# hkchengrex/Cutie

Measured on AMD Instinct MI355X. Metric: frames/sec (480p, 3 objects), higher is better.
Workload: dtype bf16

## Files before the change

cutie_amd/_lib.py:

```python
import ctypes
import os

_HERE = os.path.dirname(os.path.abspath(__file__))
LIB_PATH = os.environ.get('CUTIE_AMD_LIB') or os.path.join(_HERE, 'libcutie_hip.so')
ABI_VERSION = 9
OP_STRUCT_SIZE = 256

_lib = None


class HipLibraryError(RuntimeError):
    pass


def load():
    global _lib
    if _lib is not None:
        return _lib
    if not os.path.exists(LIB_PATH):
        raise HipLibraryError(
            f'{LIB_PATH} not found: build it with `python -c "import __graft_entry__ as g; g.build()"` '
            f'(or `make -C cutie_amd/csrc`).  cutie_amd has no CPU fallback.')
    lib = ctypes.CDLL(LIB_PATH)
    lib.cutie_exec.argtypes = [ctypes.c_void_p, ctypes.c_int, ctypes.c_void_p]
    lib.cutie_exec.restype = ctypes.c_int
    lib.cutie_exec_one.argtypes = [ctypes.c_void_p, ctypes.c_void_p]
    lib.cutie_exec_one.restype = ctypes.c_int
    lib.cutie_graph_capture.argtypes = [ctypes.c_void_p, ctypes.c_int, ctypes.c_void_p]
# ... 109 lines not shown
```

cutie_amd/csrc/api.hip:

```cpp
#include "common.h"
#include <stdarg.h>
#include <stdio.h>
#include <string.h>

static thread_local char g_err[512] = "";

void cutie_set_error(const char* fmt, ...) {
    va_list ap;
    va_start(ap, fmt);
    vsnprintf(g_err, sizeof(g_err), fmt, ap);
    va_end(ap);
}

static int dispatch(const cutie_op* op, hipStream_t s) {
    switch (op->kind) {
        case CUTIE_OP_CONV: return launch_conv(op, s);
        case CUTIE_OP_QUERY_INIT: return (op->flags & 1) ? launch_attention(op, s) : launch_elementwise(op, s);
        case CUTIE_OP_QFFN: return launch_qchain(op, s);
        case CUTIE_OP_STEM: return launch_stem(op, s);
        case CUTIE_OP_ATTN_Q2P: case CUTIE_OP_ATTN_SELF: case CUTIE_OP_ATTN_P2Q:
            return (op->flags & 12) ? launch_qchain(op, s) : launch_attention(op, s);
        case CUTIE_OP_AUX_MASK:
            return launch_attention(op, s);
        case CUTIE_OP_KEY_PREP: case CUTIE_OP_AFF_SCORE: case CUTIE_OP_AFF_SELECT: case CUTIE_OP_AFF_READOUT:
// ... 78 lines not shown
    hipGraphExecDestroy(h->exec);
    hipGraphDestroy(h->graph);
    delete h;
}

float cutie_time_ops(const cutie_op* ops, int n, int iters, void* stream) {
    hipStream_t s = (hipStream_t)stream;
    hipEvent_t a, b;
    if (hipEventCreate(&a) != hipSuccess || hipEventCreate(&b) != hipSuccess) { cutie_set_error("time: event create failed"); return -1.f; }
    if (cutie_exec(ops, n, stream) != 0) return -1.f;
    hipEventRecord(a, s);
    for (int it = 0; it < iters; ++it)
        if (cutie_exec(ops, n, stream) != 0) return -1.f;
    hipEventRecord(b, s);
    hipEventSynchronize(b);
    float ms = 0.f;
    hipEventElapsedTime(&ms, a, b);
    hipEventDestroy(a);
    hipEventDestroy(b);
    return ms / (float)iters;
}

const char* cutie_hip_last_error(void) { return g_err; }
int cutie_hip_abi_version(void) { return 9; }
int cutie_op_struct_size(void) { return (int)sizeof(cutie_op); }
int cutie_hip_build_flags(void) {
#ifdef CUTIE_DIAG
    return 1;
#else
    return 0;
#endif
}

}
```

cutie_amd/csrc/elementwise.hip:

```cpp
#include "common.h"
#include <math.h>

#define GRID1D(n, bs) dim3((unsigned)(((long)(n) + (bs) - 1) / (bs)))
__global__ void memset32_kernel(uint32_t* d, long n, uint32_t v);

__global__ void maxpool_kernel(const uint4* __restrict__ x, uint4* __restrict__ y, int B, int H, int W, int C8,
                               int OH, int OW, int relu) {
    long idx = (long)blockIdx.x * blockDim.x + threadIdx.x;
    long total = (long)B * OH * OW * C8;
    if (idx >= total) return;
    int c = idx % C8; long t = idx / C8;
    int ow = t % OW; t /= OW; int oh = t % OH; int b = t / OH;
    float m[8];
#pragma unroll
    for (int i = 0; i < 8; ++i) m[i] = relu ? 0.f : -INFINITY;
    for (int dy = 0; dy < 3; ++dy) {
        int ih = oh * 2 - 1 + dy;
        if ((unsigned)ih >= (unsigned)H) continue;
        for (int dx = 0; dx < 3; ++dx) {
            int iw = ow * 2 - 1 + dx;
            if ((unsigned)iw >= (unsigned)W) continue;
            uint4 v = x[(((long)b * H + ih) * W + iw) * C8 + c];
            uint32_t u[4] = {v.x, v.y, v.z, v.w};
#pragma unroll
// ... 344 lines not shown
                const uint32_t* xu = &xv[it].x; const uint32_t* ru = &rv[it].x;
#pragma unroll
                for (int i = 0; i < 4; ++i) {
                    const float lo = __uint_as_float(xu[i] << 16) * sc[(2 * i) * 32 + c8] + __uint_as_float(ru[i] << 16);
                    const float hi = __uint_as_float(xu[i] & 0xffff0000u) * sc[(2 * i + 1) * 32 + c8] + __uint_as_float(ru[i] & 0xffff0000u);
                    const uint32_t st = pack_bf2(lo, hi);
                    part += fmaxf(__uint_as_float(st << 16), 0.f) * __uint_as_float(wu[i] << 16);
                    part += fmaxf(__uint_as_float(st & 0xffff0000u), 0.f) * __uint_as_float(wu[i] & 0xffff0000u);
                }
            }
            part += __uint_as_float(__builtin_amdgcn_update_dpp(0, (int)__float_as_uint(part), 0xB1, 0xf, 0xf, false));
            part += __uint_as_float(__builtin_amdgcn_update_dpp(0, (int)__float_as_uint(part), 0x4E, 0xf, 0xf, false));
            part += __uint_as_float(__builtin_amdgcn_update_dpp(0, (int)__float_as_uint(part), 0x141, 0xf, 0xf, false));
            part += __uint_as_float(__builtin_amdgcn_update_dpp(0, (int)__float_as_uint(part), 0x140, 0xf, 0xf, false));
            const unsigned pu = __float_as_uint(part);
            const auto rr = __builtin_amdgcn_permlane16_swap(pu, pu, false, false);
            const float tot = __uint_as_float(rr[0]) + __uint_as_float(rr[1]);
            const int q = tid + it * 256, p = p0 + q / C8;
            if (c8 == 0 && offs[it] >= 0) plog[(long)b * HW + p] = tot + bias;
        }
    }
}

__global__ void gru4_kernel(const float* __restrict__ v, float* __restrict__ h, bf16_t* __restrict__ hb, long n, int C, int prio) {
    if (prio) __builtin_amdgcn_s_setprio(1);
    const long idx = (long)blockIdx.x * blockDim.x + threadIdx.x;
    const int C4 = C >> 2;
    if (idx >= n * C4) return;
    const long row = idx / C4; const int c = (int)(idx - row * C4) * 4;
    const float* vr = v + row * 3 * C + c;
    const float4 f4 = *reinterpret_cast<const float4*>(vr), u4 = *reinterpret_cast<const float4*>(vr + C), n4 = *reinterpret_cast<const float4*>(vr + 2 * C);
    const float4 h4 = *reinterpret_cast<const float4*>(h + row * C + c);
    const float fa[4] = {f4.x, f4.y, f4.z, f4.w}, ua[4] = {u4.x, u4.y, u4.z, u4.w}, na[4] = {n4.x, n4.y, n4.z, n4.w}, ha[4] = {h4.x, h4.y, h4.z, h4.w};
    float o[4];
#pragma unroll
    for (int i = 0; i < 4; ++i) {
        const float f = sigmoidf_(fa[i]), u = sigmoidf_(ua[i]), nv = tanhf(na[i]);
        o[i] = f * ha[i] * (1.f - u) + u * nv;
    }
    *reinterpret_cast<float4*>(h + row * C + c) = make_float4(o[0], o[1], o[2], o[3]);
    *reinterpret_cast<uint2*>(hb + row * C + c) = make_uint2(pack_bf2(o[0], o[1]), pack_bf2(o[2], o[3]));
}

__global__ void gru_kernel(const float* __restrict__ v, float* __restrict__ h, bf16_t* __restrict__ hb, long n, int C) {
    long idx = (long)blockIdx.x * blockDim.x + threadIdx.x;
    if (idx >= n * C) return;
// ... 850 lines not shown
            break;
        }
        case CUTIE_OP_MASK_DOWN: {
            int K = i[0], r = i[3], h = i[1] / r, w = i[2] / r;
            long n = (long)K * h * w;
            float* m16 = (float*)p[2];
            if (!m16) { cutie_set_error("mask_down: m16 buffer required"); return -2; }
            hipLaunchKernelGGL(mask_down_pair_kernel, GRID1D((long)h * w * 64, BS), dim3(BS), 0, s, (const float*)p[0], m16, (uint4*)p[1], K, i[1], i[2], r,
                               i[4] > 8 ? i[4] / 8 : 1);
            break;
        }
        case CUTIE_OP_GAP: {
            if (i[2] > 256 || (i[2] & 7) || 256 % (i[2] / 8)) { cutie_set_error("gap: C must divide 256 octet-wise (C=%d)", i[2]); return -2; }
            if (!p[2]) { cutie_set_error("gap: scratch buffer required"); return -2; }
            int nchunk = (i[1] + 63) / 64;
            hipLaunchKernelGGL(gap_partial_kernel, dim3(nchunk, i[0]), dim3(256), 0, s, (const bf16_t*)p[0], (float*)p[2], i[1], i[2]);
            if (!(op->flags & 1))
                hipLaunchKernelGGL(gap_final_kernel, dim3(i[0]), dim3(256), 0, s, (const float*)p[2], (float*)p[1], nchunk, i[2], 1.f / (float)i[1]);
            break;
        }
        case CUTIE_OP_ECA_APPLY: {
            if (i[2] > 256 || (i[2] & 7)) { cutie_set_error("eca: C <= 256, C %% 8"); return -2; }
            if (p[6] && (i[2] != 256 || !p[8])) { cutie_set_error("eca: the fused 1x1 head needs C = 256 and an output"); return -2; }
            int nchunk = (i[1] + 63) / 64;
            hipLaunchKernelGGL(eca_apply_kernel, dim3((i[1] + 31) / 32, i[0]), dim3(256), 0, s, (const bf16_t*)p[0], (const float*)p[5], (const float*)p[2],
                               (const bf16_t*)p[3], (bf16_t*)p[4], (float*)p[1], i[1], i[2], nchunk, (op->flags & 1) ? (const long long*)p[5] : nullptr,
                               (const bf16_t*)p[6], (const float*)p[7], (float*)p[8], PRIO);
            break;
        }
        case CUTIE_OP_GRU: {
            long n = (long)i[0] * i[1];
            if (!(op->flags & 1) && (i[1] & 3) == 0 && (((uintptr_t)p[0] | (uintptr_t)p[1]) & 15) == 0 && ((uintptr_t)p[2] & 7) == 0)
                hipLaunchKernelGGL(gru4_kernel, GRID1D(n / 4, BS), dim3(BS), 0, s, (const float*)p[0], (float*)p[1], (bf16_t*)p[2], (long)i[0], i[1], PRIO);
            else
                hipLaunchKernelGGL(gru_kernel, GRID1D(n, BS), dim3(BS), 0, s, (const float*)p[0], (float*)p[1], (bf16_t*)p[2], (long)i[0], i[1]);
            break;
        }
        case CUTIE_OP_SEG_AGG:
            hipLaunchKernelGGL(seg_agg_kernel, GRID1D(i[1], BS), dim3(BS), 0, s, (const float*)p[0], (float*)p[1], i[0], i[1]);
            break;
        case CUTIE_OP_UP4_SOFTMAX: {
            long n = (long)16 * i[1] * i[2];
            if (op->flags & 1) {
                if (i[0] > 16) { cutie_set_error("up4_softmax: the fused form holds P <= 16 planes in registers (P=%d)", i[0]); return -2; }
                const bool vec = !(op->flags & 2) && i[0] <= 8 && (((uintptr_t)p[1] | (uintptr_t)p[2]) & 15) == 0;
                const int nclip = i[4] > 1 ? i[4] : 1;
// ... 206 lines not shown
```

cutie_amd/inference/inference_core.py:

```python
import contextlib
import logging
import os
from typing import List, Optional

import numpy as np
import torch

from .. import _lib, frame_context, ops as O
from ..model import plans
from .image_feature_store import ImageFeatureStore
from .memory_manager import MemoryManager
from .object_manager import ObjectManager

log = logging.getLogger()
F32 = torch.float32
DEFER_MEM = os.environ.get('CUTIE_AMD_DEFER_MEM', '0') not in ('', '0')
WAIT_TRACE = None
AFF_BATCH = int(os.environ.get('CUTIE_AMD_AFF_BATCH', '8'))
AFF_FIRST_ALONE = os.environ.get('CUTIE_AMD_AFF_FIRST_ALONE', '1') not in ('', '0')
WINDOW = int(os.environ.get('CUTIE_AMD_WINDOW', '12'))
WINDOW_LEAD = int(os.environ.get('CUTIE_AMD_WINDOW_LEAD', '3'))


def pad_geometry(h, w, d=16):
# ... 356 lines not shown
            msk_value, finish = self.network.encode_mask(
                image, pix_feat, self.memory.get_sensory(ids), prob, deep_update=is_deep_update, chunk_size=self.chunk_size,
                need_weights=self.save_aux, _raw=raw, _split=True)
            self.memory.add_memory(key, shrinkage, msk_value, None, ids, selection=selection, as_permanent=as_permanent)
            feats = pre[2]
            ev = self._ahead_affinity(feats[2], feats[4], pre[3], self._prefetched_rec, next_mem_ti=self.curr_ti + self.mem_every, first_alone=AFF_FIRST_ALONE)
            self._prefetched = pre[:3] + (ev,) + pre[4:]
            sensory, obj_value = finish()
            self.memory.add_object_values(obj_value, ids)
        else:
            msk_value, sensory, obj_value, _ = self.network.encode_mask(
                image, pix_feat, self.memory.get_sensory(ids), prob, deep_update=is_deep_update, chunk_size=self.chunk_size,
                need_weights=self.save_aux, _raw=raw)
            self.memory.add_memory(key, shrinkage, msk_value, obj_value, ids, selection=selection, as_permanent=as_permanent)
        self.last_mem_ti = self.curr_ti
        if is_deep_update:
            self.memory.update_sensory(sensory, ids)

    def _segment(self, key, selection, pix_feat, ms_features, update_sensory=True) -> torch.Tensor:
        if not self.memory.engaged:
            log.warning('Trying to segment without any memory!')
            return torch.zeros((1, key.shape[-2] * 16, key.shape[-1] * 16), device=key.device, dtype=key.dtype)
        ids = self.object_manager.all_obj_ids
        memory_readout = self.memory.read(pix_feat, key, selection, self.last_mask, self.network)
        stacked = self.memory.readout_stacked(ids)
        memory_readout = stacked if stacked is not None else self.object_manager.realize_dict(memory_readout)
        sensory, _, pred_prob_with_bg = self.network.segment(ms_features, memory_readout, self.memory.get_sensory(ids),
                                                             chunk_size=self.chunk_size, update_sensory=update_sensory,
                                                             _need_logits=False, _fork=self._hinted)
        pred_prob_with_bg = pred_prob_with_bg[0]
        if update_sensory:
            self.memory.update_sensory(sensory, ids)
        return pred_prob_with_bg

    def step(self, image: torch.Tensor, mask: Optional[torch.Tensor] = None, objects: Optional[List[int]] = None, *,
             idx_mask: bool = True, end: bool = False, delete_buffer: bool = True, force_permanent: bool = False,
             next_image: Optional[torch.Tensor] = None, next_images=None) -> torch.Tensor:
        if objects is None and mask is not None:
            assert not idx_mask
            objects = list(range(1, mask.shape[0] + 1))

        resize_needed = False
        if self.max_internal_size > 0:
            h, w = image.shape[-2:]
            min_side = min(h, w)
            if min_side > self.max_internal_size:
                resize_needed = True
# ... 187 lines not shown
```

cutie_amd/inference/memory_manager.py:

```python
import itertools
import logging
import os
from typing import Dict, List

import torch

from .. import frame_context, ops as O
from .kv_memory_store import Bucket, StoreView, LIFE_EPS_BITS
from .object_manager import ObjectManager

log = logging.getLogger()
BF16, F32 = torch.bfloat16, torch.float32
CAND_CAP = 1024
_VALIDATE = os.environ.get('CUTIE_AMD_VALIDATE', '0') not in ('', '0')
PATCH_PLANS = os.environ.get('CUTIE_AMD_PATCH_PLANS', '1') not in ('', '0')
_VERSIONS = itertools.count(1)


class MemoryManager:
    def __init__(self, cfg, object_manager: ObjectManager):
        self.object_manager = object_manager
        self.sensory_dim = cfg.model.sensory_dim
        self.top_k = cfg.top_k
        self.chunk_size = cfg.chunk_size
# ... 407 lines not shown
                q['_readouts_joint'] = readout[e:e + C].view(C * K, h, w, m0.CV)
        return True

    def read_visual(self, q: dict, h: int, w: int, dev, network) -> Dict[int, torch.Tensor]:
        self._pool = network.engine().pool
        ahead = q.pop('_readouts', None) or {}
        ahead_ev = q.pop('_readouts_ev', None)
        if ahead_ev is not None and ahead:
            torch.cuda.current_stream(dev).wait_event(ahead_ev)
        out = {}
        for bucket in self.buckets.values():
            K = len(bucket.objects)
            pre = ahead.get(bucket.id)
            if pre is not None and pre[1] == self._version and pre[0].shape[0] == K:
                out[bucket.id] = pre[0]
                if pre[2] is not None:
                    self._commit_ahead(bucket, pre[2], network)
            else:
                self._join_side()
                out[bucket.id] = self._affinity(bucket, q, h, w, dev)
        return out

    def read(self, pix_feat: torch.Tensor, query_key: torch.Tensor, selection: torch.Tensor, last_mask: torch.Tensor,
             network) -> Dict[int, torch.Tensor]:
        q = network.query_operands(query_key, selection)
        h, w = pix_feat.shape[-2:]
        dev = pix_feat.device
        visual = self.read_visual(q, h, w, dev, network)
        all_readout = {}
        for bucket in self.buckets.values():
            K = len(bucket.objects)
            readout = visual[bucket.id]
            cs = self.chunk_size if (self.chunk_size is not None and self.chunk_size >= 1) else K
            chunks = []
            for c0 in range(0, K, cs):
                objects = bucket.objects[c0:c0 + cs]
                this_sensory = self.get_sensory(objects)
                this_last_mask = self._get_mask_by_ids(last_mask, objects)
                visual_readout = readout[c0:c0 + cs].permute(0, 3, 1, 2).unsqueeze(0)
                pixel_readout = network.pixel_fusion(pix_feat, visual_readout, this_sensory, this_last_mask)
                a, b = self._rows(objects, self._objv_ids)
                this_obj_mem = self._objv[a:b].unsqueeze(0).unsqueeze(2)
                readout_memory, aux_features = network.readout_query(pixel_readout, this_obj_mem, _last_aux=self.save_aux,
                                                                     _summary_token=(self._objv_token, a, b))
                for i, obj in enumerate(objects):
                    all_readout[obj] = readout_memory[:, i]
                chunks.append((objects, readout_memory))
                if self.save_aux:
                    self.aux = self._aux_output(this_sensory, pixel_readout, aux_features, Q=int(this_obj_mem.shape[3]))
            self._last_readout = chunks[0] if len(chunks) == 1 else (None, None)
        if _VALIDATE:
            self.check_overflow()
        return all_readout

    @staticmethod
    def _aux_output(sensory, pixel_readout, aux_features, Q: int = 16) -> dict:
        logits = [t.float().clone() for t in aux_features['logits']] if aux_features else None
        attn_mask = None
        if logits:
            lg = logits[-1]
            prob = torch.sigmoid(lg)
            bg = torch.prod(1 - prob, dim=1, keepdim=True).clamp(1e-7, 1 - 1e-7)
            pr = prob.clamp(1e-7, 1 - 1e-7)
            agg = torch.cat([torch.log(bg / (1 - bg)), torch.log(pr / (1 - pr))], 1)
            fg = agg[:, 1:] >= agg.max(dim=1, keepdim=True)[0]
            m = torch.cat([(~fg).unsqueeze(2).expand(-1, -1, Q // 2, -1, -1), fg.unsqueeze(2).expand(-1, -1, Q // 2, -1, -1)], 2).clone()
            full = m.flatten(3).all(-1)
# ... 246 lines not shown
```

cutie_amd/model/cutie.py:

```python
import logging
from typing import Dict, Iterable, List

import torch
import torch.nn as nn

from .. import _lib, frame_context
from . import plans
from .param_spec import build_spec
from .weights import fold_bn, pack_conv, pack_linear, linear_as_conv

log = logging.getLogger()
BF16, F32 = torch.bfloat16, torch.float32


def nhwc_of(t, C=None):
    p = t.permute(0, 2, 3, 1)
    if p.dtype != BF16 or not p.is_contiguous():
        p = p.to(BF16).contiguous()
    return p


def group_nhwc_of(t, dtype=BF16):
    assert t.shape[0] == 1, 'batch size 1 only (flip_aug is not supported yet)'
    p = t[0].permute(0, 2, 3, 1)
# ... 139 lines not shown
            self._pe[key] = (e.reshape(h * w, -1).float() @ self._sum_w0.t()).to(BF16).to(self.device).contiguous()
        return self._pe[key]

    def rep_embedding(self, which, K):
        key = (which, K)
        if key not in self._rep:
            e = self.sd[f'object_transformer.{which}.weight']
            self._rep[key] = e.repeat(K, 1).to(self.device).contiguous()
        return self._rep[key]

    def mask_down_bufs(self, K, h, w, clips=1):
        mb = self.__dict__.setdefault('_md_bufs', {})
        if (K, h, w, clips) not in mb:
            mb[(K, h, w, clips)] = (torch.zeros((K, h, w, 64), dtype=BF16, device=self.device), torch.zeros((K, h, w), dtype=F32, device=self.device))
        return mb[(K, h, w, clips)]

    def query_bufs(self, K):
        qb = self.__dict__.setdefault('_query_bufs', {})
        if K not in qb:
            M = K * self.m['object_transformer']['num_queries']
            qb[K] = tuple(torch.zeros((M, self.m['embed_dim']), dtype=F32, device=self.device) for _ in range(2))
        return qb[K]

    def fork(self):
        e = object.__new__(Engine)
        e.__dict__.update(self.__dict__)
        e._plans = {}
        e._arenas = {}
        e.pool = plans.SlotPool()
        e.__dict__.pop('_splitk_part', None)
        e.__dict__.pop('_streams', None)
        e.__dict__.pop('_query_bufs', None)
        e.__dict__.pop('_md_bufs', None)
        e.__dict__.pop('_qinit_state', None)
        return e

    def plan(self, key, builder, *args):
        p = self._plans.get(key)
        if p is None:
            p = builder(self, *args)
            p.ol.finalize()
            kind = 'side' if key[0] in ('enc', 'key') else ('win' if key[0] == 'encw' else 'main')
            arenas = self.__dict__.setdefault('_arenas', {})
            if kind not in arenas:
                arenas[kind] = plans.Arena(self.device)
            p.pack_into(arenas[kind])
            self._plans[key] = p
        return p

# ... 286 lines not shown
                frame_context.remember('sensory_bf16', sf, sb)
                return group_logical(sf), summ.unsqueeze(0)
            return group_logical(value), finish
        P.run(**dyn)
        new_sens = group_logical(sf)
        frame_context.remember('sensory_bf16', sf, sb)
        return group_logical(value), new_sens, summ.unsqueeze(0), None

    def pixel_fusion(self, pix_feat, pixel, sensory, last_mask, *, chunk_size=-1):
        eng = self.engine()
        pf = nhwc_of(pix_feat)
        px = group_nhwc_of(pixel)
        K, h, w = px.shape[:3]
        _, sb = self._sensory_pair(sensory)
        lm = f32c(last_mask[0])
        xt = frame_context.recall('fuse_xt', pf)
        md = frame_context.recall('mask_down', lm)
        md = md is not None and md == (K, h, w, eng.__dict__.get('_md_gen'))
        P = eng.plan(('fuse', K, h, w, xt is not None, md), plans.build_pixel_fusion, K, h, w, xt is not None, md)
        fused = eng.pool.get(('fuse', K, h, w, eng.devstr), dict(fused=((K, h, w, self.embed_dim), BF16, False)), eng.device)['fused']
        P.run(pix_feat=pf, pixel=px, sensory_bf16=sb, last_mask=lm, fused=fused, **({} if xt is None else {'fuse_xt': xt}))
        return group_logical(fused)

    def readout_query(self, pixel_readout, obj_memory, *, selector=None, need_weights=False, _last_aux=True, _summary_token=None):
        assert selector is None, 'selector is a training-time argument'
        eng = self.engine()
        px = group_nhwc_of(pixel_readout)
        K, h, w = px.shape[:3]
        om = obj_memory[0]
        if om.dtype != F32:
            om = om.to(F32)
        om = om.sum(dim=1) if om.shape[1] != 1 else om[:, 0]
        if not om.is_contiguous():
            om = om.contiguous()
        st = eng.__dict__.setdefault('_qinit_state', {})
        fresh = _summary_token is None or st.get(K) != _summary_token or not plans.QINIT_SKIP
        st[K] = _summary_token
        P = eng.plan(('rq', K, h, w, bool(_last_aux), fresh), plans.build_readout_query, K, h, w, bool(_last_aux), fresh)
        out = eng.pool.get(('rq', K, h, w, eng.devstr), dict(out=((K, h, w, self.embed_dim), BF16, False)), eng.device)['out']
        P.run(pixel=px, obj_mem=om, out=out)
        n_aux = P.bufs['aux_logits'].shape[0] - (0 if _last_aux else 1)
        aux = {'logits': [P.bufs['aux_logits'][i].view(1, K, h, w) for i in range(n_aux)],
               'q_weights': None, 'p_weights': None}
        return group_logical(out), aux

    def segment(self, ms_image_feat: List[torch.Tensor], memory_readout, sensory, *, selector=None, chunk_size=-1,
                update_sensory=True, _need_logits=True, _fork=False):
        assert selector is None, 'selector is a training-time argument'
        eng = self.engine()
        dev = eng.device
        p16 = group_nhwc_of(memory_readout)
        K, h, w = p16.shape[:3]
        f8, f4 = nhwc_of(ms_image_feat[1]), nhwc_of(ms_image_feat[2])
        sf, sb = self._sensory_pair(sensory)
        pre = frame_context.recall('decoder_feats', f8)
        if pre is not None and pre[2].data_ptr() != f4.data_ptr():
            pre = None
        md = bool(_fork) and K + 1 <= 8 and dev.type == 'cuda'
        P = eng.plan(('seg', K, h, w, bool(update_sensory), pre is not None, md), plans.build_segment, K, h, w, bool(update_sensory), pre is not None, md)
        sp = dict(prob=((K + 1, 16 * h, 16 * w), F32, False))
        if _need_logits:
            sp['lup'] = ((K + 1, 16 * h, 16 * w), F32, False)
        o = eng.pool.get(('seg', K, h, w, bool(_need_logits), eng.devstr), sp, dev)
        prob, lup = o['prob'], o.get('lup')
        feats = dict(f8=f8, f4=f4) if pre is None else dict(f8p=pre[0], f4p=pre[1])
        dyn = dict(p16=p16, sensory_f32=sf, sensory_bf16=sb, prob=prob, logits_up=lup, **feats)
        n_ops, cut = len(P.ol.recs), P.meta.get('logits_done', 0)
        if _fork and not eng.one_lane and update_sensory and dev.type == 'cuda' and not plans.GRAPHS and 0 < cut < n_ops - 1 and K + 1 <= 16:
            main = torch.cuda.current_stream(dev)
            st = eng.__dict__.setdefault('_streams', {})
            if 'aux' not in st:
                st['aux'] = torch.cuda.Stream(device=dev)
            aux = st['aux']
            P.run_part(0, cut, **dyn)
            aux.wait_stream(main)
            with torch.cuda.stream(aux):
                P.run_part(n_ops - 1, n_ops, first=False)
            P.run_part(cut, n_ops - 1, first=False)
            main.wait_stream(aux)
        else:
            P.run(**dyn)
        new_sens = group_logical(sf)
# ... 17 lines not shown
```

cutie_amd/model/plans.py:

```python
import math
import os

import numpy as np
import torch

from .. import _lib
from .. import ops as O
from ..ops import Dyn
from .param_spec import resnet_layers

BF16, F32 = torch.bfloat16, torch.float32


class Act:
    __slots__ = ('t', 'B', 'H', 'W', 'C', 'ld')

    def __init__(self, t, B, H, W, C, ld=None):
        self.t, self.B, self.H, self.W, self.C, self.ld = t, B, H, W, C, (C if ld is None else ld)


def positional_encoding(h, w, dim_total, scale, temperature):
    dim = int(math.ceil(dim_total / 4) * 2)
    inv_freq = 1.0 / (temperature ** (torch.arange(0, dim, 2).float() / dim))
    py = torch.arange(h, dtype=torch.float32)
# ... 322 lines not shown
            save_tile_cache(cache)

    def conv(self, wname, x, *, name=None, out=None, stride=1, pad=None, x2=None, res=None, res_bcast=False,
             relu_in=False, act=O.ACT_NONE, out_f32=False, ldy=None, gap_acc=None, zero=None, persistent=False, res_group=None):
        w = self.eng.w[wname]
        if pad is None:
            pad = (w.kh - 1) // 2
        OH = (x.H + 2 * pad - w.kh) // stride + 1
        OW = (x.W + 2 * pad - w.kw) // stride + 1
        if out is None:
            t = self.buf(name or wname, (x.B, OH, OW, w.cout), F32 if out_f32 else BF16, persistent=persistent)
            out = Act(t, x.B, OH, OW, w.cout, w.cout if ldy is None else ldy)
        else:
            assert out.B == x.B and out.H == OH and out.W == OW and out.C == w.cout, (wname, out.B, out.H, out.W, out.C, OH, OW, w.cout)
        if res is not None:
            assert res.C == w.cout and res.H == OH and res.W == OW
        self.ol.conv(x.t, w, out.t, B=x.B, H=x.H, W=x.W, C1=x.C, ldx1=x.ld, OH=OH, OW=OW, ldy=out.ld, stride=stride,
                     pad=pad, x2=None if x2 is None else x2.t, C2=0 if x2 is None else x2.C,
                     ldx2=0 if x2 is None else x2.ld, res=None if res is None else res.t,
                     ldr=0 if res is None else res.ld, res_bcast=res_bcast, relu_in=relu_in, act=act, out_f32=out_f32,
                     gap_acc=gap_acc, zero=zero, prio=self.prio, res_group=res_group)
        return out

    def ca_block(self, prefix, x, name, out=None, head=None):
        if head is not None:
            head = (self.eng.w[head[0]], head[1])
        w = self.eng.w[prefix + '.conv2']
        gap = self.buf(name + '.gap', (x.B, x.C), F32)
        HW = x.H * x.W
        if O.conv_side_jobs_ok(cin=x.C, cout=w.cout, kh=w.kh):
            sums = self.buf(name + '.gapsum', (x.B, x.C), torch.int64)
            t1 = self.conv(prefix + '.conv1', x, name=name + '.t1', relu_in=True, act=O.ACT_RELU, zero=sums)
            t2 = self.conv(prefix + '.conv2', t1, name=name + '.t2', gap_acc=sums)
            if out is None:
                out = Act(self.buf(name + '.out', (x.B, x.H, x.W, x.C)), x.B, x.H, x.W, x.C)
            self.ol.eca_apply(t2.t, gap, self.eng.w[prefix + '.conv.weight'], x.t, out.t, B=x.B, HW=HW, C=x.C, fixed_sums=sums, head=head)
            return out
        t1 = self.conv(prefix + '.conv1', x, name=name + '.t1', relu_in=True, act=O.ACT_RELU)
        t2 = self.conv(prefix + '.conv2', t1, name=name + '.t2')
        self.ol.gap(t2.t, gap, B=x.B, HW=HW, C=x.C, partial_only=True)
        if out is None:
            out = Act(self.buf(name + '.out', (x.B, x.H, x.W, x.C)), x.B, x.H, x.W, x.C)
        self.ol.eca_apply(t2.t, gap, self.eng.w[prefix + '.conv.weight'], x.t, out.t, B=x.B, HW=HW, C=x.C, head=head)
        return out

    def fusion_block(self, prefix, x, g, name, out=None, xt=None, xt_group=None):
        if xt is None:
            xt = self.conv(prefix + '.distributor.x_transform', x, name=name + '.xt')
        g0 = self.conv(prefix + '.distributor.g_transform', g, name=name + '.g0', res=xt, res_bcast=True, res_group=xt_group)
        g1 = self.ca_block(prefix + '.block1', g0, name + '.b1')
        return self.ca_block(prefix + '.block2', g1, name + '.b2', out=out)

    def resnet(self, prefix, x, taps=None):
        bottleneck, layers = resnet_layers(self.eng.m, prefix)
        feats = {}
        for (lname, planes, nb, lstride) in layers:
            for bi in range(nb):
                p = f'{prefix}.{lname}.{bi}'
                s = lstride if bi == 0 else 1
                last = bi == nb - 1
# ... 85 lines not shown
        P.ol.keep.append(pair)
    else:
        pair = P.buf('pair', (K, h, w, 64), persistent=True)
        m16 = P.buf('m16', (K, h, w), F32)
        for c in range(G):
            P.ol.mask_down(Dyn('last_mask' if G == 1 else 'last_mask%d' % c), pair[c * Kc:], m16[c * Kc:], K=Kc, H=16 * h, W=16 * w, pair_channels=64)
    if G > 1 and not stacked:
        px = P.buf('pixel_all', (K, h, w, m['value_dim']))
        nb = Kc * h * w * m['value_dim'] * 2
        P.ol.bank_write([(Dyn('pixel%d' % c), px[c * Kc:], nb) for c in range(G)])
        pixel = Act(px, K, h, w, m['value_dim'])
    else:
        pixel = Act(Dyn('pixel'), K, h, w, m['value_dim'])
    p16 = P.conv('pixel_fuser.sensory_compress', Act(Dyn('sensory_bf16'), K, h, w, m['sensory_dim']),
                 x2=Act(pair, K, h, w, 64), res=pixel, name='p16')
    xt = Act(Dyn('fuse_xt'), G, h, w, eng.w['pixel_fuser.fuser.distributor.x_transform'].cout) if pre else None
    P.fusion_block('pixel_fuser.fuser', Act(Dyn('pix_feat'), 1, h, w, m['pixel_dim']), p16, 'fuse',
                   out=Act(Dyn('fused'), K, h, w, m['embed_dim']), xt=xt, xt_group=(Kc, wstride * h * w) if G > 1 else None)
    if G > 1:
        P.korder_ref = G
    return P


def build_readout_query(eng, K, h, w, last_aux=True, fresh=True, clips=1):
    G, Kc = clips, K
    K = G * Kc
    P = Plan(eng, touch=weights_go_cold(h * w, K))
    if G > 1:
        P.korder_ref = G
    m, ol, W = eng.m, P.ol, eng.w
    ot = m['object_transformer']
    C, Q, heads, nb = m['embed_dim'], ot['num_queries'], ot['num_heads'], ot['num_blocks']
    HW, M = h * w, K * Q
    t = 'object_transformer'
    f = lambda name, shape: P.buf(name, shape, F32)
    query, query_emb = eng.query_bufs(K)
    use_chain = C == 256 and Q == 16 and heads == 8 and HW <= 24576 and ot['ff_dim'] % 64 == 0
    assert G == 1 or use_chain, 'clips in lock step need the chain form of the query side'
    qacc = P.buf('qacc', (3 * nb, M, C), torch.int64) if use_chain else None
    zero_on_conv = None
    if C == 256 and Q == 16:
        if fresh or not use_chain:
            ol.query_init2(Dyn('obj_mem'), query, query_emb, rows=M, w_init=W[t + '.summary_to_query_init'], res_init=eng.rep_embedding('query_init', K),
                           w_emb=W[t + '.summary_to_query_emb'], res_emb=eng.rep_embedding('query_emb', K), zero=qacc)
        elif O.conv_side_jobs_ok(cin=C, cout=C, kh=1):
            zero_on_conv = qacc
        else:
            ol.memset32(qacc, 2 * qacc.numel(), 0)
    else:
# ... 66 lines not shown
            sa = f(n + 'sa', (M, C))
            if fuse_proj:
                ol.attn_self(None, None, sa, K=K, Q=Q, C=C, heads=heads,
                             proj=dict(x=x1, W=W[q + '.self_attn.qkv'], emb=query_emb, ln=ln('.self_attn.norm'), ln_out=y))
            else:
                qkv = f(n + 'qkv', (M, 3 * C))
                ol.linear(x1, W[q + '.self_attn.qkv'], qkv, M=M, x_add=query_emb, add_rows=M, add_cols=2 * C, ln=ln('.self_attn.norm'), ln_out=y)
                ol.attn_self(qkv, qkv.view(-1)[2 * C:], sa, K=K, Q=Q, C=C, heads=heads, ldqk=3 * C, ldv=3 * C)
            x2 = f(n + 'x2', (M, C))
            ol.linear(sa, W[q + '.self_attn.out'], x2, M=M, res=y)
            hid = f(n + 'hid', (M, ot['ff_dim']))
            ol.linear(x2, W[q + '.ffn.linear1'], hid, M=M, relu=True, ln=ln('.ffn.norm'))
            x3 = f(n + 'x3', (M, C))
            ol.linear(hid, W[q + '.ffn.linear2'], x3, M=M, res=x2)
            x = x3
            pa = P.buf(n + 'pa', (K, h, w, C))
            if fuse_proj:
                ol.attn_p2q(kvq.t.view(-1)[2 * C:], None, None, pa, K=K, Q=Q, HW=HW, C=C, heads=heads, ldq=3 * C,
                            proj=dict(x=x, W=W[q + '.read_from_query.kv'], emb=query_emb))
            else:
                kv2 = f(n + 'kv2', (M, 2 * C))
                ol.linear(x, W[q + '.read_from_query.kv'], kv2, M=M, x_add=query_emb, add_rows=M, add_cols=C)
                ol.attn_p2q(kvq.t.view(-1)[2 * C:], kv2, kv2.view(-1)[C:], pa, K=K, Q=Q, HW=HW, C=C, heads=heads, ldq=3 * C, ldkv=2 * C)
        pf = P.conv(q + '.read_from_query.out', Act(pa, K, h, w, C), name=n + 'pf', res=pixel)
        last = b == nb - 1
        want_aux = not last or last_aux
        fuse_head = want_aux and C == 256
        pixel = P.ca_block(q + '.pixel_ffn.conv', pf, n + 'ffn', out=Act(Dyn('out'), K, h, w, C) if last else None,
                           head=(f'{t}.mask_pred.{b + 1}.1', aux[b + 1]) if fuse_head else None)
        if want_aux and not fuse_head:
            P.conv(f'{t}.mask_pred.{b + 1}.1', pixel, relu_in=True, out_f32=True, out=Act(aux[b + 1], K, h, w, 1))
        if not last and not fused_mask:
            ol.aux_mask(aux[b + 1], fg, nfg, K=K, HW=HW)
    return P


def build_segment(eng, K, h, w, update_sensory, pre=False, md=False, clips=1, wstride=1):
    G, Kc = clips, K
    K = G * Kc
    assert G == 1 or (pre and Kc + 1 <= 8), 'clips in lock step: image-only decoder convs from the encoder plan, <= 7 objects per clip'
    P = Plan(eng, touch=weights_go_cold(h * w, K))
    if G > 1:
        P.korder_ref = G
    m, ol = eng.m, P.ol
    up = m['mask_decoder']['up_dims']
    ms = m['pixel_encoder']['ms_dims']
    CS = m['sensory_dim']
    h8, w8, h4, w4 = 2 * h, 2 * w, 4 * h, 4 * w
    if pre:
        f8p, f4p = Act(Dyn('f8p'), G, h8, w8, up[0]), Act(Dyn('f4p'), G, h4, w4, up[1])
    else:
        f8p = P.conv('mask_decoder.decoder_feat_proc.transforms.0', Act(Dyn('f8'), 1, h8, w8, ms[1]), name='f8p')
        f4p = P.conv('mask_decoder.decoder_feat_proc.transforms.1', Act(Dyn('f4'), 1, h4, w4, ms[2]), name='f4p')
    p16 = Act(Dyn('p16'), K, h, w, up[0])
    u8 = P.buf('u8', (K, h8, w8, up[0]))
    ol.upsample2x_add(p16.t, f8p.t, u8, B=K, h=h, w=w, C=up[0], skip_group=(Kc, wstride * h8 * w8) if G > 1 else None)
    u8 = Act(u8, K, h8, w8, up[0])
    t1 = P.conv('mask_decoder.up_16_8.out_conv.conv1', u8, relu_in=True, act=O.ACT_RELU)
    ds = P.conv('mask_decoder.up_16_8.out_conv.downsample', u8)
    p8 = P.conv('mask_decoder.up_16_8.out_conv.conv2', t1, res=ds, name='p8')
    u4 = P.buf('u4', (K, h4, w4, up[1]))
    ol.upsample2x_add(p8.t, f4p.t, u4, B=K, h=h8, w=w8, C=up[1], skip_group=(Kc, wstride * h4 * w4) if G > 1 else None)
    u4 = Act(u4, K, h4, w4, up[1])
    t2 = P.conv('mask_decoder.up_8_4.out_conv.conv1', u4, relu_in=True, act=O.ACT_RELU)
    p4 = P.conv('mask_decoder.up_8_4.out_conv.conv2', t2, res=u4, name='p4')
    logits = P.buf('logits', (K, h4, w4), F32)
    P.conv('mask_decoder.pred', p4, relu_in=True, out_f32=True, out=Act(logits, K, h4, w4, 1))
    P.meta['logits_done'] = len(ol.recs)
    if update_sensory:
        CT = up[1] + up[2] + 64
        gcat = P.buf('gcat', (K, h, w, CT), persistent=True)
        ol.area_down3([dict(x=p8.t, y=gcat, B=K, H=h8, W=w8, C=up[1], ldx=up[1], ldy=CT, r=2),
                       dict(x=p4.t, y=gcat.view(-1)[up[1]:], B=K, H=h4, W=w4, C=up[2], ldx=up[2], ldy=CT, r=4),
                       dict(x=logits, y=gcat.view(-1)[up[1] + up[2]:], B=K, H=h4, W=w4, C=1, ldx=1, ldy=CT, r=4, f32_in=True, Cz=8)])
        g3 = P.conv('mask_decoder.sensory_update.g_all', p16, x2=Act(gcat, K, h, w, CT), name='g3')
        vals = P.conv('mask_decoder.sensory_update.transform', g3, x2=Act(Dyn('sensory_bf16'), K, h, w, CS),
                      out_f32=True, name='gru_vals')
        ol.gru(vals.t, Dyn('sensory_f32'), Dyn('sensory_bf16'), n=K * h * w, C=CS)
    if Kc + 1 <= 16:
# ... 72 lines not shown
```

cutie_amd/ops.py:

```python
import os

import numpy as np
import torch

from . import _lib

NI, NF, NP = 24, 6, 16
OP_DTYPE = np.dtype([('kind', '<i4'), ('flags', '<i4'), ('i', '<i4', (NI,)), ('f', '<f4', (NF,)), ('p', '<u8', (NP,))])
assert OP_DTYPE.itemsize == _lib.OP_STRUCT_SIZE

(CONV, MAXPOOL, IMG_PREP, UPSAMPLE2X_ADD, AREA_DOWN, MASK_DOWN, GAP, ECA_APPLY, GRU, SEG_AGG, UP4_SOFTMAX,
 MASK_MERGE, AGG_SOFTMAX, LINEAR, LAYERNORM, QUERY_INIT, AUX_MASK, ATTN_Q2P, ATTN_SELF, ATTN_P2Q, SUMMARIZE,
 ADD_PE, KEY_PREP, AFF_SCORE, AFF_SELECT, AFF_READOUT, MEMSET32, COPY2D, AXPY, USAGE_TICK, RANK_SELECT,
 GATHER_ROWS, CONSOL_AFF, CONSOL_READ, CAST, PROB_TO_ID, RESIZE, FLIP_W, AREA_DOWN3, QFFN, STEM, BANK_WRITE) = range(1, 43)

KIND_NAMES = {}
for _n in ('CONV MAXPOOL IMG_PREP UPSAMPLE2X_ADD AREA_DOWN MASK_DOWN GAP ECA_APPLY GRU SEG_AGG UP4_SOFTMAX MASK_MERGE '
           'AGG_SOFTMAX LINEAR LAYERNORM QUERY_INIT AUX_MASK ATTN_Q2P ATTN_SELF ATTN_P2Q SUMMARIZE ADD_PE KEY_PREP '
           'AFF_SCORE AFF_SELECT AFF_READOUT MEMSET32 COPY2D AXPY USAGE_TICK RANK_SELECT GATHER_ROWS CONSOL_AFF '
           'CONSOL_READ CAST PROB_TO_ID RESIZE FLIP_W AREA_DOWN3 QFFN STEM').split():
    KIND_NAMES[globals()[_n]] = _n

F_RELU_IN, F_OUT_F32, F_RES_BCAST = 1, 2, 4
F_PRIO, F_AFF_PRIO = 256, 64
# ... 404 lines not shown

    def mask_down(self, masks, pair, m16, *, K, H, W, r=16, pair_channels=8):
        assert pair_channels % 8 == 0
        return self.add(MASK_DOWN, 0, [K, H, W, r, pair_channels], [], [masks, pair, m16])

    def gap(self, x, y, *, B, HW, C, scratch=None, partial_only=False):
        if scratch is None:
            scratch = torch.zeros((B, -(-HW // 64), C), dtype=torch.float32, device=y.device)
        self._last_gap_scratch = scratch
        return self.add(GAP, 1 if partial_only else 0, [B, HW, C], [], [x, y, scratch])

    def eca_apply(self, x, gap, wk, r, y, *, B, HW, C, part=None, fixed_sums=None, head=None):
        tail = []
        if head is not None:
            w, out = head
            assert C == 256 and w.cout == 1 and w.kh == 1 and w.cin_padded == 256
            tail = [w.weight, w.bias, out]
        if fixed_sums is not None:
            return self.add(ECA_APPLY, 1, [B, HW, C], [], [x, gap, wk, r, y, fixed_sums] + tail)
        if part is None:
            part = self._last_gap_scratch
        return self.add(ECA_APPLY, 0, [B, HW, C], [], [x, gap, wk, r, y, part] + tail)

    def gru(self, values, h, hb, *, n, C):
        return self.add(GRU, GRU_SCALAR, [n, C], [], [values, h, hb])

    def seg_agg(self, logits, agg, *, K, hw):
        return self.add(SEG_AGG, 0, [K, hw], [], [logits, agg])

    def up4_softmax(self, agg, prob, logits_up, *, P, h, w, from_logits=False, mask_down=None, clips=1):
        if mask_down is not None:
            assert from_logits and P <= 8 and h % 4 == 0 and w % 4 == 0
            m16, pair, pitch = mask_down
            return self.add(UP4_SOFTMAX, 1 | 4 | UP4_RTK | UP4_LANES, [P, h, w, pitch, clips], [], [agg, prob, logits_up, m16, pair])
        assert clips == 1 or (from_logits and P <= 8)
        return self.add(UP4_SOFTMAX, (1 | UP4_RTK) if from_logits else 0, [P, h, w, 0, clips], [], [agg, prob, logits_up])

    def mask_merge(self, inmask, pred, src, planes, *, h0, w0, H, W, pad_left, pad_top, Knew, Kold, nfloat, float_mode):
        return self.add(MASK_MERGE, 1 if float_mode else 0, [h0, w0, H, W, pad_left, pad_top, Knew, Kold, nfloat], [],
                        [inmask, pred, src, planes])

    def agg_softmax(self, planes, prob, *, K, HW):
        return self.add(AGG_SOFTMAX, 0, [K, HW], [], [planes, prob])

    def linear(self, x, w, y, *, M, ldx=None, ldy=None, x_add=None, add_rows=0, res=None, relu=False, add_cols=0,
               ln=None, ln_out=None, eps=1e-5):
# ... 328 lines not shown
```

Baseline: 1164.

## Defer final ECA apply into segment's upsample2x-add kernel

The last object-transformer block's ECA channel-attention apply is now skipped at the end of readout_query when a single bucket is read in one chunk without aux output. It is fused into a new eca_up2x kernel in the segment plan that applies the ECA, writes the readout, and produces the 2x bilinear upsample plus skip add in one pass. The aim is to drop one kernel launch and one full write-then-read of the readout activation. In exchange, state (handover buffers and a generation counter) is shared across plans. Each thread also re-reads neighbouring pixels and recomputes the sigmoid scales per block.

```diff
diff --git a/cutie_amd/_lib.py b/cutie_amd/_lib.py
--- a/cutie_amd/_lib.py
+++ b/cutie_amd/_lib.py
@@ -3,7 +3,7 @@
 
 _HERE = os.path.dirname(os.path.abspath(__file__))
 LIB_PATH = os.environ.get('CUTIE_AMD_LIB') or os.path.join(_HERE, 'libcutie_hip.so')
-ABI_VERSION = 9
+ABI_VERSION = 10
 OP_STRUCT_SIZE = 256
 
 _lib = None
diff --git a/cutie_amd/csrc/api.hip b/cutie_amd/csrc/api.hip
--- a/cutie_amd/csrc/api.hip
+++ b/cutie_amd/csrc/api.hip
@@ -124,7 +124,7 @@
 }
 
 const char* cutie_hip_last_error(void) { return g_err; }
-int cutie_hip_abi_version(void) { return 9; }
+int cutie_hip_abi_version(void) { return 10; }
 int cutie_op_struct_size(void) { return (int)sizeof(cutie_op); }
 int cutie_hip_build_flags(void) {
 #ifdef CUTIE_DIAG
diff --git a/cutie_amd/csrc/elementwise.hip b/cutie_amd/csrc/elementwise.hip
--- a/cutie_amd/csrc/elementwise.hip
+++ b/cutie_amd/csrc/elementwise.hip
@@ -390,6 +390,95 @@
     }
 }
 
+__device__ __forceinline__ uint4 up2x_tap(const uint4* yv, const uint4& sk, int oy, int ox, int h, int w) {
+    int y0, y1, x0, x1; float ly, lx;
+    up_coord(oy, h, 0.5f, y0, y1, ly);
+    up_coord(ox, w, 0.5f, x0, x1, lx);
+    const uint32_t* a = &yv[0].x; const uint32_t* bq = &yv[1].x; const uint32_t* cq = &yv[2].x; const uint32_t* d = &yv[3].x;
+    const uint32_t* s = &sk.x;
+    float w00 = (1.f - ly) * (1.f - lx), w01 = (1.f - ly) * lx, w10 = ly * (1.f - lx), w11 = ly * lx;
+    uint32_t out[4];
+#pragma unroll
+    for (int i = 0; i < 4; ++i) {
+        float lo = w00 * __uint_as_float(a[i] << 16) + w01 * __uint_as_float(bq[i] << 16) +
+                   w10 * __uint_as_float(cq[i] << 16) + w11 * __uint_as_float(d[i] << 16) + __uint_as_float(s[i] << 16);
+        float hi = w00 * __uint_as_float(a[i] & 0xffff0000u) + w01 * __uint_as_float(bq[i] & 0xffff0000u) +
+                   w10 * __uint_as_float(cq[i] & 0xffff0000u) + w11 * __uint_as_float(d[i] & 0xffff0000u) +
+                   __uint_as_float(s[i] & 0xffff0000u);
+        out[i] = pack_bf2(lo, hi);
+    }
+    return make_uint4(out[0], out[1], out[2], out[3]);
+}
+
+__global__ __launch_bounds__(256) void eca_up2x_kernel(const bf16_t* __restrict__ x, const long long* __restrict__ fixed,
+                                                       const float* __restrict__ wk, const bf16_t* __restrict__ r, bf16_t* __restrict__ y,
+                                                       float* __restrict__ gap_out, const uint4* __restrict__ skip, uint4* __restrict__ u,
+                                                       int h, int w, int C, int Kg, long gstride, int prio) {
+    if (prio) __builtin_amdgcn_s_setprio(1);
+    __shared__ float gap[256 + 4], sc[256];
+    const int b = blockIdx.y, tid = threadIdx.x;
+    const int HW = h * w, C8 = C >> 3, OH = 2 * h, OW = 2 * w;
+    const float inv = 1.f / (float)HW;
+    const int pp = tid / C8, c8 = tid - pp * C8, p = blockIdx.x * (256 / C8) + pp;
+    const bool ok = p < HW;
+    const int iy = ok ? p / w : 0, ix = ok ? p - iy * w : 0;
+    const int iy1 = min(iy + 1, h - 1), ix1 = min(ix + 1, w - 1);
+    const long o00 = ((long)b * HW + (long)iy * w + ix) * C + c8 * 8;
+    const long offs[4] = {o00, ((long)b * HW + (long)iy * w + ix1) * C + c8 * 8, ((long)b * HW + (long)iy1 * w + ix) * C + c8 * 8,
+                          ((long)b * HW + (long)iy1 * w + ix1) * C + c8 * 8};
+    uint4 xv[4], rv[4], sk[4];
+#pragma unroll
+    for (int k = 0; k < 4; ++k) {
+        xv[k] = *reinterpret_cast<const uint4*>(x + offs[k]);
+        rv[k] = *reinterpret_cast<const uint4*>(r + offs[k]);
+    }
+    const uint4* sb = skip + (Kg > 0 ? (b / Kg) * gstride : 0l) * C8 + c8;
+    uint4* ub = u + (long)b * OH * OW * C8 + c8;
+#pragma unroll
+    for (int k = 0; k < 4; ++k) {
+        const int oy = min(2 * iy + 1 + (k >> 1), OH - 1), ox = min(2 * ix + 1 + (k & 1), OW - 1);
+        sk[k] = sb[((long)oy * OW + ox) * C8];
+    }
+    for (int c = tid; c < C; c += 256) {
+        const float mean = (float)((double)fixed[(long)b * C + c] * (1.0 / 16777216.0)) * inv;
+        gap[c + 2] = mean;
+        if (gap_out && blockIdx.x == 0) gap_out[(long)b * C + c] = mean;
+    }
+    if (tid < 2) { gap[tid] = 0.f; gap[C + 2 + tid] = 0.f; }
+    __syncthreads();
+    for (int c = tid; c < C; c += 256) {
+        float a = wk[0] * gap[c] + wk[1] * gap[c + 1] + wk[2] * gap[c + 2] + wk[3] * gap[c + 3] + wk[4] * gap[c + 4];
+        sc[(c & 7) * 32 + (c >> 3)] = sigmoidf_(a);
+    }
+    __syncthreads();
+    if (!ok) return;
+    uint4 yv[4];
+#pragma unroll
+    for (int k = 0; k < 4; ++k) {
+        const uint32_t* xu = &xv[k].x; const uint32_t* ru = &rv[k].x;
+        uint32_t o[4];
+#pragma unroll
+        for (int i = 0; i < 4; ++i) {
+            float lo = __uint_as_float(xu[i] << 16) * sc[(2 * i) * 32 + c8] + __uint_as_float(ru[i] << 16);
+            float hi = __uint_as_float(xu[i] & 0xffff0000u) * sc[(2 * i + 1) * 32 + c8] + __uint_as_float(ru[i] & 0xffff0000u);
+            o[i] = pack_bf2(lo, hi);
+        }
+        yv[k] = make_uint4(o[0], o[1], o[2], o[3]);
+    }
+    *reinterpret_cast<uint4*>(y + o00) = yv[0];
+#pragma unroll
+    for (int k = 0; k < 4; ++k) {
+        const int oy = 2 * iy + 1 + (k >> 1), ox = 2 * ix + 1 + (k & 1);
+        if (oy < OH && ox < OW) ub[((long)oy * OW + ox) * C8] = up2x_tap(yv, sk[k], oy, ox, h, w);
+    }
+    if (iy == 0)
+        for (int ox = ix == 0 ? 0 : 2 * ix + 1; ox <= min(2 * ix + 2, OW - 1); ++ox)
+            ub[(long)ox * C8] = up2x_tap(yv, sb[(long)ox * C8], 0, ox, h, w);
+    if (ix == 0)
+        for (int oy = 2 * iy + 1; oy <= min(2 * iy + 2, OH - 1); ++oy)
+            ub[(long)oy * OW * C8] = up2x_tap(yv, sb[(long)oy * OW * C8], oy, 0, h, w);
+}
+
 __global__ void gru4_kernel(const float* __restrict__ v, float* __restrict__ h, bf16_t* __restrict__ hb, long n, int C, int prio) {
     if (prio) __builtin_amdgcn_s_setprio(1);
     const long idx = (long)blockIdx.x * blockDim.x + threadIdx.x;
@@ -1286,6 +1375,18 @@
         case CUTIE_OP_ECA_APPLY: {
             if (i[2] > 256 || (i[2] & 7)) { cutie_set_error("eca: C <= 256, C %% 8"); return -2; }
             if (p[6] && (i[2] != 256 || !p[8])) { cutie_set_error("eca: the fused 1x1 head needs C = 256 and an output"); return -2; }
+            if (op->flags & 2) {
+                const int C8 = i[2] / 8;
+                if (!(op->flags & 1) || p[6] || i[2] < 8 || 256 % C8 || i[3] < 1 || i[4] < 1 || (long)i[3] * i[4] != i[1] || !p[9] || !p[10]) {
+                    cutie_set_error("eca+up2x: needs the conv's fixed-point sums, no head, C/8 dividing 256, h * w = HW, a skip map and an output"); return -2;
+                }
+                if (p[4] == p[0] || p[4] == p[3]) { cutie_set_error("eca+up2x: y must not alias x or r (neighbouring threads read them)"); return -2; }
+                if (i[5] < 0 || (i[5] > 0 && (i[0] % i[5] || i[6] < 4 * i[3] * i[4]))) { cutie_set_error("eca+up2x: skip groups of %d objects do not divide B = %d (or their stride is below one map)", i[5], i[0]); return -2; }
+                const int ppb = 256 / C8;
+                hipLaunchKernelGGL(eca_up2x_kernel, dim3((i[1] + ppb - 1) / ppb, i[0]), dim3(256), 0, s, (const bf16_t*)p[0], (const long long*)p[5], (const float*)p[2],
+                                   (const bf16_t*)p[3], (bf16_t*)p[4], (float*)p[1], (const uint4*)p[9], (uint4*)p[10], i[3], i[4], i[2], i[5], (long)i[6], PRIO);
+                break;
+            }
             int nchunk = (i[1] + 63) / 64;
             hipLaunchKernelGGL(eca_apply_kernel, dim3((i[1] + 31) / 32, i[0]), dim3(256), 0, s, (const bf16_t*)p[0], (const float*)p[5], (const float*)p[2],
                                (const bf16_t*)p[3], (bf16_t*)p[4], (float*)p[1], i[1], i[2], nchunk, (op->flags & 1) ? (const long long*)p[5] : nullptr,
diff --git a/cutie_amd/inference/inference_core.py b/cutie_amd/inference/inference_core.py
--- a/cutie_amd/inference/inference_core.py
+++ b/cutie_amd/inference/inference_core.py
@@ -402,7 +402,7 @@
             log.warning('Trying to segment without any memory!')
             return torch.zeros((1, key.shape[-2] * 16, key.shape[-1] * 16), device=key.device, dtype=key.dtype)
         ids = self.object_manager.all_obj_ids
-        memory_readout = self.memory.read(pix_feat, key, selection, self.last_mask, self.network)
+        memory_readout = self.memory.read(pix_feat, key, selection, self.last_mask, self.network, _segment_next=ids)
         stacked = self.memory.readout_stacked(ids)
         memory_readout = stacked if stacked is not None else self.object_manager.realize_dict(memory_readout)
         sensory, _, pred_prob_with_bg = self.network.segment(ms_features, memory_readout, self.memory.get_sensory(ids),
diff --git a/cutie_amd/inference/memory_manager.py b/cutie_amd/inference/memory_manager.py
--- a/cutie_amd/inference/memory_manager.py
+++ b/cutie_amd/inference/memory_manager.py
@@ -453,7 +453,7 @@
         return out
 
     def read(self, pix_feat: torch.Tensor, query_key: torch.Tensor, selection: torch.Tensor, last_mask: torch.Tensor,
-             network) -> Dict[int, torch.Tensor]:
+             network, *, _segment_next=None) -> Dict[int, torch.Tensor]:
         q = network.query_operands(query_key, selection)
         h, w = pix_feat.shape[-2:]
         dev = pix_feat.device
@@ -463,6 +463,8 @@
             K = len(bucket.objects)
             readout = visual[bucket.id]
             cs = self.chunk_size if (self.chunk_size is not None and self.chunk_size >= 1) else K
+            defer = (_segment_next is not None and len(self.buckets) == 1 and cs >= K and not self.save_aux
+                     and list(bucket.objects) == list(_segment_next))
             chunks = []
             for c0 in range(0, K, cs):
                 objects = bucket.objects[c0:c0 + cs]
@@ -473,7 +475,7 @@
                 a, b = self._rows(objects, self._objv_ids)
                 this_obj_mem = self._objv[a:b].unsqueeze(0).unsqueeze(2)
                 readout_memory, aux_features = network.readout_query(pixel_readout, this_obj_mem, _last_aux=self.save_aux,
-                                                                     _summary_token=(self._objv_token, a, b))
+                                                                     _summary_token=(self._objv_token, a, b), _defer_eca=defer)
                 for i, obj in enumerate(objects):
                     all_readout[obj] = readout_memory[:, i]
                 chunks.append((objects, readout_memory))
diff --git a/cutie_amd/model/cutie.py b/cutie_amd/model/cutie.py
--- a/cutie_amd/model/cutie.py
+++ b/cutie_amd/model/cutie.py
@@ -185,9 +185,19 @@
             qb[K] = tuple(torch.zeros((M, self.m['embed_dim']), dtype=F32, device=self.device) for _ in range(2))
         return qb[K]
 
+    def eca_handover_bufs(self, K, h, w):
+        eb = self.__dict__.setdefault('_eca_bufs', {})
+        if (K, h, w) not in eb:
+            C = self.m['embed_dim']
+            eb[(K, h, w)] = dict(t2=torch.zeros((K, h, w, C), dtype=BF16, device=self.device), x=torch.zeros((K, h, w, C), dtype=BF16, device=self.device),
+                                 sums=torch.zeros((K, C), dtype=torch.int64, device=self.device), gap=torch.zeros((K, C), dtype=F32, device=self.device))
+        return eb[(K, h, w)]
+
     def fork(self):
         e = object.__new__(Engine)
         e.__dict__.update(self.__dict__)
+        e.__dict__.pop('_eca_bufs', None)
+        e.__dict__.pop('_eca_gen', None)
         e._plans = {}
         e._arenas = {}
         e.pool = plans.SlotPool()
@@ -520,7 +530,8 @@
         P.run(pix_feat=pf, pixel=px, sensory_bf16=sb, last_mask=lm, fused=fused, **({} if xt is None else {'fuse_xt': xt}))
         return group_logical(fused)
 
-    def readout_query(self, pixel_readout, obj_memory, *, selector=None, need_weights=False, _last_aux=True, _summary_token=None):
+    def readout_query(self, pixel_readout, obj_memory, *, selector=None, need_weights=False, _last_aux=True, _summary_token=None,
+                      _defer_eca=False):
         assert selector is None, 'selector is a training-time argument'
         eng = self.engine()
         px = group_nhwc_of(pixel_readout)
@@ -534,9 +545,15 @@
         st = eng.__dict__.setdefault('_qinit_state', {})
         fresh = _summary_token is None or st.get(K) != _summary_token or not plans.QINIT_SKIP
         st[K] = _summary_token
-        P = eng.plan(('rq', K, h, w, bool(_last_aux), fresh), plans.build_readout_query, K, h, w, bool(_last_aux), fresh)
+        defer = bool(_defer_eca) and not _last_aux and eng.device.type == 'cuda' and plans.eca_defer_ok(eng)
+        P = eng.plan(('rq', K, h, w, bool(_last_aux), fresh, defer), plans.build_readout_query, K, h, w, bool(_last_aux), fresh, 1, defer)
         out = eng.pool.get(('rq', K, h, w, eng.devstr), dict(out=((K, h, w, self.embed_dim), BF16, False)), eng.device)['out']
         P.run(pixel=px, obj_mem=om, out=out)
+        if defer:
+            eng._eca_gen = eng.__dict__.get('_eca_gen', 0) + 1
+            frame_context.remember('eca_deferred', out, (K, h, w, eng._eca_gen), cap=2)
+        else:
+            frame_context.forget('eca_deferred', out)
         n_aux = P.bufs['aux_logits'].shape[0] - (0 if _last_aux else 1)
         aux = {'logits': [P.bufs['aux_logits'][i].view(1, K, h, w) for i in range(n_aux)],
                'q_weights': None, 'p_weights': None}
@@ -555,7 +572,15 @@
         if pre is not None and pre[2].data_ptr() != f4.data_ptr():
             pre = None
         md = bool(_fork) and K + 1 <= 8 and dev.type == 'cuda'
-        P = eng.plan(('seg', K, h, w, bool(update_sensory), pre is not None, md), plans.build_segment, K, h, w, bool(update_sensory), pre is not None, md)
+        eca = frame_context.recall('eca_deferred', p16)
+        if eca is not None:
+            frame_context.forget('eca_deferred', p16)
+            if eca != (K, h, w, eng.__dict__.get('_eca_gen')):
+                raise RuntimeError('segment: this read-out was returned by readout_query(_defer_eca=True) and another such call has run since; '
+                                   'its last launch can no longer be made')
+        eca = eca is not None
+        P = eng.plan(('seg', K, h, w, bool(update_sensory), pre is not None, md, eca), plans.build_segment, K, h, w, bool(update_sensory), pre is not None, md,
+                     1, 1, eca)
         sp = dict(prob=((K + 1, 16 * h, 16 * w), F32, False))
         if _need_logits:
             sp['lup'] = ((K + 1, 16 * h, 16 * w), F32, False)
diff --git a/cutie_amd/model/plans.py b/cutie_amd/model/plans.py
--- a/cutie_amd/model/plans.py
+++ b/cutie_amd/model/plans.py
@@ -368,13 +368,18 @@
                      gap_acc=gap_acc, zero=zero, prio=self.prio, res_group=res_group)
         return out
 
-    def ca_block(self, prefix, x, name, out=None, head=None):
+    def ca_block(self, prefix, x, name, out=None, head=None, defer=None):
         if head is not None:
             head = (self.eng.w[head[0]], head[1])
         w = self.eng.w[prefix + '.conv2']
         gap = self.buf(name + '.gap', (x.B, x.C), F32)
         HW = x.H * x.W
         if O.conv_side_jobs_ok(cin=x.C, cout=w.cout, kh=w.kh):
+            if defer is not None:
+                assert head is None and out is None and x.t is defer['x']
+                t1 = self.conv(prefix + '.conv1', x, name=name + '.t1', relu_in=True, act=O.ACT_RELU, zero=defer['sums'])
+                self.conv(prefix + '.conv2', t1, out=Act(defer['t2'], x.B, x.H, x.W, x.C), gap_acc=defer['sums'])
+                return None
             sums = self.buf(name + '.gapsum', (x.B, x.C), torch.int64)
             t1 = self.conv(prefix + '.conv1', x, name=name + '.t1', relu_in=True, act=O.ACT_RELU, zero=sums)
             t2 = self.conv(prefix + '.conv2', t1, name=name + '.t2', gap_acc=sums)
@@ -382,6 +387,7 @@
                 out = Act(self.buf(name + '.out', (x.B, x.H, x.W, x.C)), x.B, x.H, x.W, x.C)
             self.ol.eca_apply(t2.t, gap, self.eng.w[prefix + '.conv.weight'], x.t, out.t, B=x.B, HW=HW, C=x.C, fixed_sums=sums, head=head)
             return out
+        assert defer is None, 'a deferred ECA needs the channel sums of the conv (eca_defer_ok)'
         t1 = self.conv(prefix + '.conv1', x, name=name + '.t1', relu_in=True, act=O.ACT_RELU)
         t2 = self.conv(prefix + '.conv2', t1, name=name + '.t2')
         self.ol.gap(t2.t, gap, B=x.B, HW=HW, C=x.C, partial_only=True)
@@ -513,9 +519,17 @@
     return P
 
 
-def build_readout_query(eng, K, h, w, last_aux=True, fresh=True, clips=1):
+def eca_defer_ok(eng):
+    C = eng.m['embed_dim']
+    w = eng.w['object_transformer.blocks.%d.pixel_ffn.conv.conv2' % (eng.m['object_transformer']['num_blocks'] - 1)]
+    return (not _lib.get_executor().is_mock and C == eng.m['mask_decoder']['up_dims'][0] and C % 8 == 0 and C <= 256 and 256 % (C // 8) == 0
+            and O.conv_side_jobs_ok(cin=C, cout=w.cout, kh=w.kh))
+
+
+def build_readout_query(eng, K, h, w, last_aux=True, fresh=True, clips=1, defer_eca=False):
     G, Kc = clips, K
     K = G * Kc
+    assert not defer_eca or (not last_aux and eca_defer_ok(eng))
     P = Plan(eng, touch=weights_go_cold(h * w, K))
     if G > 1:
         P.korder_ref = G
@@ -628,8 +642,13 @@
                 kv2 = f(n + 'kv2', (M, 2 * C))
                 ol.linear(x, W[q + '.read_from_query.kv'], kv2, M=M, x_add=query_emb, add_rows=M, add_cols=C)
                 ol.attn_p2q(kvq.t.view(-1)[2 * C:], kv2, kv2.view(-1)[C:], pa, K=K, Q=Q, HW=HW, C=C, heads=heads, ldq=3 * C, ldkv=2 * C)
+        last = b == nb - 1
+        if last and defer_eca:
+            hb = eng.eca_handover_bufs(K, h, w)
+            pf = P.conv(q + '.read_from_query.out', Act(pa, K, h, w, C), out=Act(hb['x'], K, h, w, C), res=pixel)
+            P.ca_block(q + '.pixel_ffn.conv', pf, n + 'ffn', defer=hb)
+            break
         pf = P.conv(q + '.read_from_query.out', Act(pa, K, h, w, C), name=n + 'pf', res=pixel)
-        last = b == nb - 1
         want_aux = not last or last_aux
         fuse_head = want_aux and C == 256
         pixel = P.ca_block(q + '.pixel_ffn.conv', pf, n + 'ffn', out=Act(Dyn('out'), K, h, w, C) if last else None,
@@ -641,7 +660,7 @@
     return P
 
 
-def build_segment(eng, K, h, w, update_sensory, pre=False, md=False, clips=1, wstride=1):
+def build_segment(eng, K, h, w, update_sensory, pre=False, md=False, clips=1, wstride=1, eca=False):
     G, Kc = clips, K
     K = G * Kc
     assert G == 1 or (pre and Kc + 1 <= 8), 'clips in lock step: image-only decoder convs from the encoder plan, <= 7 objects per clip'
@@ -660,7 +679,13 @@
         f4p = P.conv('mask_decoder.decoder_feat_proc.transforms.1', Act(Dyn('f4'), 1, h4, w4, ms[2]), name='f4p')
     p16 = Act(Dyn('p16'), K, h, w, up[0])
     u8 = P.buf('u8', (K, h8, w8, up[0]))
-    ol.upsample2x_add(p16.t, f8p.t, u8, B=K, h=h, w=w, C=up[0], skip_group=(Kc, wstride * h8 * w8) if G > 1 else None)
+    if eca:
+        hb = eng.eca_handover_bufs(K, h, w)
+        wk = eng.w['object_transformer.blocks.%d.pixel_ffn.conv.conv.weight' % (m['object_transformer']['num_blocks'] - 1)]
+        ol.eca_apply_up2x(hb['t2'], hb['gap'], wk, hb['x'], p16.t, f8p.t, u8, B=K, h=h, w=w, C=up[0], fixed_sums=hb['sums'],
+                          skip_group=(Kc, wstride * h8 * w8) if G > 1 else None)
+    else:
+        ol.upsample2x_add(p16.t, f8p.t, u8, B=K, h=h, w=w, C=up[0], skip_group=(Kc, wstride * h8 * w8) if G > 1 else None)
     u8 = Act(u8, K, h8, w8, up[0])
     t1 = P.conv('mask_decoder.up_16_8.out_conv.conv1', u8, relu_in=True, act=O.ACT_RELU)
     ds = P.conv('mask_decoder.up_16_8.out_conv.downsample', u8)
diff --git a/cutie_amd/ops.py b/cutie_amd/ops.py
--- a/cutie_amd/ops.py
+++ b/cutie_amd/ops.py
@@ -450,6 +450,12 @@
             part = self._last_gap_scratch
         return self.add(ECA_APPLY, 0, [B, HW, C], [], [x, gap, wk, r, y, part] + tail)
 
+    def eca_apply_up2x(self, x, gap, wk, r, y, skip, u, *, B, h, w, C, fixed_sums, skip_group=None):
+        assert C % 8 == 0 and C <= 256 and 256 % (C // 8) == 0, C
+        kg, stride = (0, 0) if skip_group is None else (int(skip_group[0]), int(skip_group[1]))
+        assert skip_group is None or (kg > 0 and B % kg == 0 and stride >= 4 * h * w)
+        return self.add(ECA_APPLY, 1 | 2, [B, h * w, C, h, w, kg, stride], [], [x, gap, wk, r, y, fixed_sums, None, None, None, skip, u])
+
     def gru(self, values, h, hb, *, n, C):
         return self.add(GRU, GRU_SCALAR, [n, C], [], [values, h, hb])
 
```

After: 1163. About the same (-0.1%).
